# zcash/halo2

Measured on NVIDIA H100. Metric: msm_pairs_per_s, higher is better.
Workload: dtype u32x8 (255-bit modular integers)

## Files before the change

halo2_b200/csrc/capi_msm.cu:

```cuda
#define H2_MSM_QUAD_ACCUM_REFS (g_ctx.small_accum_refs)
#include "util_kernels.cuh"
#include "msm.cuh"
#include "ipa.cuh"
#include "ntt.cuh"
#include "ecfft.cuh"
#include "fixedbase.cuh"
static_assert(H2_FB_BITS == H2_FB_BITS_CTX, "ctx.cuh: fixed_table");


static int exclusive_scan_u32(uint32_t *d, uint64_t n, cudaStream_t s, const uint32_t *only_if = nullptr) {
    const uint64_t per_block = (uint64_t)H2_SCAN_BLOCK * H2_SCAN_ITEMS;
    uint32_t nb = (uint32_t)((n + per_block - 1) / per_block);
    if (g_ctx.scan_blocks.ensure((size_t)nb * 4 + 16)) return 1;
    uint32_t *bs = g_ctx.scan_blocks.as<uint32_t>();
    LAUNCH(scan_block_sums_kernel, nb, H2_SCAN_BLOCK, 0, s, d, n, bs, only_if);
    LAUNCH(scan_single_block_kernel, 1, H2_SCAN_BLOCK, 0, s, bs, nb, only_if);
    LAUNCH(scan_apply_kernel, nb, H2_SCAN_BLOCK, 0, s, d, n, bs, only_if);
    return 0;
}

uint32_t g_chunk_cut[H2_MAX_UPLOAD_CHUNKS + 1][H2_MAX_UPLOAD_CHUNKS + 1] = {
    {0, 16, 16, 16, 16}, {0, 16, 16, 16, 16}, {0, 4, 16, 16, 16}, {0, 2, 8, 16, 16}, {0, 1, 4, 10, 16}};
static inline size_t chunk_first(size_t n, uint32_t k, uint32_t j) {
    const auto &cut = g_chunk_cut;
// ... 28 lines not shown
        ge = &X.graphs.back();
    }
    ge->stamp = ++X.graph_stamp;
    if (ge->exec) {
        CU(cudaGraphLaunch(ge->exec, s));
        g_launches.fetch_add(ge->launches, std::memory_order_relaxed);
        return 0;
    }
    if (ge->seen++ == 0) return issue();
    const uint64_t l0 = g_launches.load();
    if (cudaStreamBeginCapture(s, cudaStreamCaptureModeThreadLocal) != cudaSuccess) { cudaGetLastError(); return issue(); }
    int rc = issue();
    cudaGraph_t graph = nullptr;
    cudaError_t ce = cudaStreamEndCapture(s, &graph);
    if (rc || ce != cudaSuccess || !graph) {
        if (graph) cudaGraphDestroy(graph);
        cudaGetLastError();
        ge->seen = 0;
        return rc ? rc : issue();
    }
    ge->launches = g_launches.load() - l0;
    ce = cudaGraphInstantiate(&ge->exec, graph, 0);
    cudaGraphDestroy(graph);
    if (ce != cudaSuccess) { ge->exec = nullptr; cudaGetLastError(); return issue(); }
    CU(cudaGraphLaunch(ge->exec, s));
    return 0;
}

template <class P, class PS>
static int msm_run(const fe *d_scalars, int scalars_mont, const affine *d_bases, size_t n, uint32_t c, uint32_t fixed, uint64_t stride,
                   jacobian *d_out, int out_canonical, cudaStream_t s, const BasesChunks *bc = nullptr, uint32_t sets = 1) {
    Context &X = g_ctx;
    if (n == 0) {
        jacobian id;
        id.x = fe_zero(); id.y = out_canonical ? fe_zero() : fe_one<P>(); id.z = fe_zero();
        if (out_canonical) id.y.v[0] = 1;
        std::vector<jacobian> ids(sets ? sets : 1u, id);
        CU(cudaMemcpyAsync(d_out, ids.data(), ids.size() * sizeof id, cudaMemcpyHostToDevice, s));
        CU(cudaStreamSynchronize(s));
        return 0;
    }
    std::function<int()> issue;
    auto record = [&X](uint32_t mode, uint32_t c_, uint32_t W, uint32_t sets_, uint32_t accum, uint32_t natural, uint32_t fast) {
        const uint32_t v[8] = {mode, c_, W, sets_, accum, natural, fast, X.fast_retry ? 1u : 0u};
        memcpy(X.last_plan, v, sizeof v);
        X.have_plan = true;
    };
    if (fixed == 2) {
        FbPlan fp;
        fp.total = n; fp.sets = sets ? sets : 1u; fp.split = fb_split(n, fp.sets); fp.scalars_mont = scalars_mont ? 1u : 0u;
        record(2, H2_FB_BITS, H2_FB_WINDOWS, fp.sets, 2, 0, 0);
        const uint64_t count0 = n * fp.split;
        if (X.fb_a.ensure(fp.sets * count0 * sizeof(xyzz)) || X.fb_b.ensure(fp.sets * fb_ctas(count0, fb_fan(count0)) * sizeof(xyzz))) return 1;
        issue = [&X, fp, count0, d_scalars, d_bases, d_out, out_canonical, s]() -> int {
            auto k_acc = fb_accum_kernel<P, PS>;
            auto k_red = fb_reduce_kernel<P, PS>;
            xyzz *a = X.fb_a.as<xyzz>(), *b = X.fb_b.as<xyzz>();
            prof_begin(PROF_MSM_ACCUM0, s);
            LAUNCH(k_acc, blocks_for(fp.sets * count0, 128), 128, 0, s, fp, d_scalars, d_bases, a);
            prof_end(s);
            uint64_t count = count0, in_stride = count0;
            for (;;) {
                const uint32_t f = fb_fan(count);
                const uint64_t ctas = fb_ctas(count, f);
                LAUNCH(k_red, dim3((unsigned)ctas, fp.sets), 4 * H2_FB_QUADS, 0, s, (const xyzz *)a, count, in_stride, f, b, ctas,
                       ctas == 1 ? d_out : (jacobian *)nullptr, (uint32_t)out_canonical);
                if (ctas == 1) break;
                xyzz *t = a; a = b; b = t;
                count = ctas; in_stride = ctas;
            }
            return 0;
        };
        return msm_issue_or_replay(issue, !bc, d_scalars, d_bases, d_out, n, stride, H2_FB_BITS, fp.sets, scalars_mont, out_canonical, s);
    }
    const uint32_t glv = (!fixed && X.glv_on && n < (1ull << 30)) ? 1u : 0u;
    if (c == 0) c = X.window_override ? X.window_override : msm_default_window(n, glv);
    if (c > 24) return fail("msm: window bits > 24");
    const uint32_t K = (bc && !fixed && bc->k > 1) ? bc->k : 1u;
    const uint32_t force_cap = X.sort_bins ? 0u : H2_MSM_NO_BINS;
    MsmPlan p;
    msm_make_plan(p, n, c, 0, 0, fixed, stride, glv, sets, force_cap);
    p.chunks = K;
    p.fast = (fixed == 1 && !bc && X.fast_now && p.cap != 0) ? 1u : 0u;
    X.last_fast = p.fast != 0;
    if (p.fast && p.T < p.cap) { p.T = p.cap; p.acc_chunk[0] = p.T; }
    p.natural = (p.fast && p.G <= X.natural_max_buckets && p.max_refs <= 2 * H2_MSM_QUAD_ACCUM_REFS && (X.accum_ways <= 1 || X.accum_ways >= 12)) ? 1u : 0u;
    MsmPlan pk[H2_MAX_UPLOAD_CHUNKS];
    size_t first[H2_MAX_UPLOAD_CHUNKS + 1];
    for (uint32_t j = 0; j <= K; j++) first[j] = chunk_first(n, K, j);
    uint64_t ref_space = 0, max_items = 0, part_total = 0;
    uint32_t t_max = 0;
    for (uint32_t j = 0; j < K; j++) {
        if (K == 1) pk[0] = p;
        else msm_make_plan(pk[j], first[j + 1] - first[j], c, 0, 0, fixed, stride, glv, sets, force_cap);
        if (pk[j].ref_space >= (1ull << 32)) return fail("msm: n * windows exceeds 2^32 references");
        ref_space = pk[j].ref_space > ref_space ? pk[j].ref_space : ref_space;
        max_items = pk[j].max_items > max_items ? pk[j].max_items : max_items;
        part_total = pk[j].part_total > part_total ? pk[j].part_total : part_total;
        t_max = pk[j].T > t_max ? pk[j].T : t_max;
    }
    bool thread_per_item = false;
    for (uint32_t j = 0; j < K; j++) thread_per_item |= pk[j].max_refs > (pk[j].fixed ? 2 : 1) * H2_MSM_QUAD_ACCUM_REFS;
    record(fixed, c, p.W, p.sets, thread_per_item ? 1u : 0u, p.natural, p.fast);
    uint64_t ba_space = 0;
    if (!fixed && X.ba_rounds) {
        size_t free_b = 0, total_b = 0;
        CU(cudaMemGetInfo(&free_b, &total_b));
        for (uint32_t j = 0; j < K; j++) {
            if (pk[j].max_refs > H2_MSM_QUAD_ACCUM_REFS && (uint64_t)K * pk[j].ref_space * 56 <= free_b / 2) msm_plan_ba(pk[j], X.ba_rounds, X.ba_target);
            if (pk[j].ba) ba_space = pk[j].ref_space > ba_space ? pk[j].ref_space : ba_space;
        }
    }
    if (K == 1) p.ba = pk[0].ba;
    if (ba_space)
        for (uint32_t r = 0; r < H2_BA_MAX_ROUNDS; r++)
            if (X.ba_lv[r].ensure(K * ((ba_space >> (r + 1)) + 1) * sizeof(affine))) return 1;
    if (glv && (X.bases_phi.ensure(n * sizeof(affine)) || X.glv_parts.ensure(n * 32))) return 1;
    if (fixed && (uint64_t)p.W * stride >= (1ull << 31)) return fail("msm: window table too large for 31-bit references");
    if (p.G >= (1ull << 32) || n >= (1ull << 31)) return fail("msm: n * windows exceeds 2^32 references");
    if (scalars_mont && X.scal_canon.ensure(n * p.sets * sizeof(fe))) return 1;
    const size_t small_words = 2 * (t_max + 2) + 8;
    part_total += 1;
    if (X.counts.ensure(K * (p.G + 1) * 4) || X.cursor.ensure(K * 2 * p.G * 4) || X.refs.ensure(K * ref_space * 4) ||
        X.size_hist.ensure(K * small_words * 4) || X.items.ensure(K * max_items * sizeof(uint2)) ||
        X.bucket_sum.ensure(K * p.G * sizeof(xyzz)) || X.pkey.ensure(K * part_total * 4) || X.pstart.ensure(K * part_total * 4) ||
        X.pend.ensure(K * part_total * 4) || X.ppt.ensure(K * part_total * sizeof(xyzz)) ||
        X.ra_t.ensure((size_t)p.Wb * p.m1 * sizeof(xyzz)) || X.ra_e.ensure((size_t)p.Wb * p.m1 * sizeof(xyzz)) ||
        X.r0.ensure((size_t)p.Wb * p.nb0 * H2_R0_ROWS * sizeof(xyzz)) || X.r1.ensure((size_t)p.Wb * p.r1_rows * sizeof(xyzz)) ||
        X.wsum.ensure((size_t)p.Wb * sizeof(xyzz)))
        return 1;
    MsmBuffers Mk[H2_MAX_UPLOAD_CHUNKS];
    for (uint32_t j = 0; j < K; j++) {
        MsmBuffers &M = Mk[j];
        const size_t o = first[j];
        M.scalars = d_scalars + o; M.bases = d_bases + o; M.bases_phi = X.bases_phi.as<affine>() + o;
        M.glv_parts = X.glv_parts.as<uint32_t>() + 8 * o; M.scalars_mont = scalars_mont ? 1u : 0u;
        M.scal_canon = X.scal_canon.as<fe>() + o;
        M.counts = X.counts.as<uint32_t>() + j * (p.G + 1); M.cursor = X.cursor.as<uint32_t>() + j * 2 * p.G; M.cursor2 = M.cursor + p.G;
        M.refs = X.refs.as<uint32_t>() + j * ref_space;
        M.size_hist = X.size_hist.as<uint32_t>() + j * small_words; M.size_cursor = M.size_hist + (pk[j].T + 2); M.flags = M.size_cursor + (pk[j].T + 2);
        M.items = X.items.as<uint2>() + j * max_items;
        M.bucket_sum = X.bucket_sum.as<xyzz>() + j * p.G;
        for (uint32_t r = 0; r < H2_BA_MAX_ROUNDS; r++) M.ba[r] = ba_space ? X.ba_lv[r].as<affine>() + j * ((ba_space >> (r + 1)) + 1) : nullptr;
        M.pkey = X.pkey.as<uint32_t>() + j * part_total; M.pstart = X.pstart.as<uint32_t>() + j * part_total;
        M.pend = X.pend.as<uint32_t>() + j * part_total; M.ppt = X.ppt.as<xyzz>() + j * part_total;
        M.ra_t = X.ra_t.as<xyzz>(); M.ra_e = X.ra_e.as<xyzz>(); M.r0 = X.r0.as<xyzz>(); M.r1 = X.r1.as<xyzz>();
        M.wsum = X.wsum.as<xyzz>(); M.result = d_out;
    }
    X.last_flags = Mk[0].flags;

    {
        const uint64_t per_block = (uint64_t)H2_SCAN_BLOCK * H2_SCAN_ITEMS;
        if (X.scan_blocks.ensure((size_t)((p.G + 1 + per_block - 1) / per_block) * 4 + 16)) return 1;
    }
    issue = [&]() -> int {
        if (!p.fast) CU(cudaMemsetAsync(X.counts.p, 0, K * (p.G + 1) * 4, s));
        CU(cudaMemsetAsync(X.cursor.p, 0, K * 2 * p.G * 4, s));
        CU(cudaMemsetAsync(X.size_hist.p, 0, K * small_words * 4, s));
        CU(cudaMemsetAsync(X.bucket_sum.p, 0, K * p.G * sizeof(xyzz), s));
        if (!p.fast) CU(cudaMemsetAsync(X.pkey.p, 0xff, K * part_total * 4, s));

        auto k_bin = msm_bin_kernel<P, PS>;
        auto k_hist = msm_hist_kernel<P, PS>;
        auto k_scatter = msm_scatter_kernel<P, PS>;
        auto k_ihist = msm_item_hist_kernel<P, PS>;
        auto k_ibases = msm_item_bases_kernel<P, PS>;
        auto k_iplace = msm_item_place_kernel<P, PS>;
        auto k_accum0 = msm_accum0_kernel<P, PS>;
        auto k_accum0q = msm_accum0_quad_kernel<P, PS>;
        auto k_accum0p2 = msm_accum0_pair_kernel<P, PS>;
        auto k_accum0s2 = msm_accum0_split_kernel<P, PS, 2>;
        auto k_accum0s4 = msm_accum0_split_kernel<P, PS, 4>;
        auto k_accum0m2 = msm_accum0_multi_kernel<P, PS, 2>;
        auto k_accum0m4 = msm_accum0_multi_kernel<P, PS, 4>;
        auto k_ba = X.ba_variant == 1 ? msm_ba_round_kernel<P, PS, 4, 5> : X.ba_variant == 2 ? msm_ba_round_kernel<P, PS, 2, 4>
                  : X.ba_variant == 3 ? msm_ba_round_kernel<P, PS, 2, 5> : msm_ba_round_kernel<P, PS, 4, 4>;
        auto k_accum0p = msm_accum0_pts_kernel<P, PS>;
        auto k_accumN = msm_accumN_kernel<P, PS>;
        auto k_rest = msm_accum_rest_kernel<P, PS>;
        auto k_reduceA = msm_reduceA_kernel<P, PS>;
        auto k_r0 = msm_r0_kernel<P, PS>;
        auto k_r1 = msm_r1_kernel<P, PS>;
        auto k_wsum = msm_wsum_kernel<P, PS>;
        auto k_final = msm_final_kernel<P, PS>;
        for (uint32_t j = 0; j < K; j++) {
            const MsmPlan &q = pk[j];
            const MsmBuffers &M = Mk[j];
            if (bc && bc->k) {
                for (uint32_t e = (K > 1 ? j : 0); e < (K > 1 ? j + 1 : bc->k); e++) {
                    if (bc->wait_recorded(2 * e + 1)) return fail("msm: the upload of the inputs failed");
                    CU(cudaStreamWaitEvent(s, bc->ev_scal[e], 0));
                }
            }
            if (q.cap == 0) CU(cudaMemsetAsync(M.flags + 1, 0x01, 4, s));
            else LAUNCH(k_bin, blocks_for(q.n * q.sets, 256), 256, 0, s, q, M);
            if (!q.fast) {
                LAUNCH(k_hist, blocks_for(q.n * q.sets, 256), 256, 0, s, q, M);
                if (exclusive_scan_u32(M.counts, q.G + 1, s, M.flags + 1)) return 1;
                LAUNCH(k_scatter, blocks_for(q.n * q.sets, 256), 256, 0, s, q, M);
            }
            if (!q.natural) {
                LAUNCH(k_ihist, blocks_for(q.G, 256), 256, 0, s, q, M);
                LAUNCH(k_ibases, 1, 32, 0, s, q, M);
                LAUNCH(k_iplace, blocks_for(q.G, 256), 256, 0, s, q, M);
            }
            if (bc && bc->k) {
                for (uint32_t e = (K > 1 ? j : 0); e < (K > 1 ? j + 1 : bc->k); e++) {
                    if (bc->wait_recorded(2 * e + 2)) return fail("msm: the upload of the inputs failed");
                    CU(cudaStreamWaitEvent(s, bc->ev[e], 0));
                }
            }
            if (q.glv) {
                auto k_phi = msm_phi_kernel<P, PS>;
                LAUNCH(k_phi, blocks_for(q.n, 256), 256, 0, s, M.bases, M.bases_phi, (uint64_t)q.n);
            }
            prof_begin(PROF_MSM_ACCUM0, s);
            if (q.max_refs <= (q.fixed ? 2 : 1) * H2_MSM_QUAD_ACCUM_REFS) {
                if (X.accum_ways == 4) LAUNCH(k_accum0m4, blocks_for(q.max_items * 16, 128), 128, 0, s, q, M);
                else if (X.accum_ways == 2) LAUNCH(k_accum0m2, blocks_for(q.max_items * 8, 128), 128, 0, s, q, M);
                else if (X.accum_ways == 0) LAUNCH(k_accum0p2, blocks_for(q.max_items * 2, 128), 128, 0, s, q, M);
                else if (X.accum_ways == 12) LAUNCH(k_accum0s2, blocks_for(q.max_items * 2, 128), 128, 0, s, q, M);
                else if (X.accum_ways == 14) LAUNCH(k_accum0s4, blocks_for(q.max_items * 4, 128), 128, 0, s, q, M);
                else LAUNCH(k_accum0q, blocks_for(q.max_items * 4, 128), 128, 0, s, q, M);
            }
            else {
                for (uint32_t r = 1; r <= q.ba; r++)
                    LAUNCH(k_ba, blocks_for((q.max_items + q.ba_m[r - 1] - 1) / q.ba_m[r - 1], 128), 128, 0, s, q, M, r);
                if (q.ba) LAUNCH(k_accum0p, blocks_for(q.max_items, 128), 128, 0, s, q, M);
                LAUNCH(k_accum0, blocks_for(q.max_items, 128), 128, 0, s, q, M);
            }
            prof_end(s);
            if (!q.fast) {
                if (q.acc_levels > 1) LAUNCH(k_accumN, blocks_for(q.acc_threads[1], 128), 128, 0, s, q, M, 1u);
                if (q.acc_levels > 2) LAUNCH(k_accumN, blocks_for(q.acc_threads[2], 128), 128, 0, s, q, M, 2u);
                if (q.acc_levels > 3) LAUNCH(k_rest, 1, 256, 0, s, q, M);
            }
        }
        const MsmBuffers &M = Mk[0];
        LAUNCH(k_reduceA, blocks_for((uint64_t)p.Wb * p.m1 * 4, 128), 128, 0, s, p, M);
        LAUNCH(k_r0, blocks_for((uint64_t)p.Wb * p.nb0 * (2 + p.bits0) * 4, 128), 128, 0, s, p, M);
        LAUNCH(k_r1, p.Wb * p.r1_rows, 4 * H2_R1_QUADS, 0, s, p, M);
        LAUNCH(k_wsum, p.Wb, 128, 0, s, p, M);
        LAUNCH(k_final, 1, 64, 0, s, p, M, (uint32_t)out_canonical);
        return 0;
    };
    return msm_issue_or_replay(issue, fixed && !bc, d_scalars, d_bases, d_out, n, stride, c, sets, scalars_mont, out_canonical, s);
}

int msm_dispatch(int curve, const fe *d_scalars, int scalars_mont, const affine *d_bases, size_t n, uint32_t c,
                 jacobian *d_out, int out_canonical, cudaStream_t s, uint32_t fixed, uint64_t stride,
                 const BasesChunks *bc, uint32_t sets) {
    if (curve == H2_CURVE_PALLAS) return msm_run<FpParams, FqParams>(d_scalars, scalars_mont, d_bases, n, c, fixed, stride, d_out, out_canonical, s, bc, sets);
    if (curve == H2_CURVE_VESTA) return msm_run<FqParams, FpParams>(d_scalars, scalars_mont, d_bases, n, c, fixed, stride, d_out, out_canonical, s, bc, sets);
    return fail("unknown curve id");
}
int fixed_pass_flags(cudaStream_t s) {
    Context &X = g_ctx;
    if (!X.last_fast) return 0;
    if (!X.h_flags) CU(cudaHostAlloc((void **)&X.h_flags, 2 * sizeof(uint32_t), cudaHostAllocDefault));
    CU(cudaMemcpyAsync(X.h_flags, X.last_flags, 2 * sizeof(uint32_t), cudaMemcpyDeviceToHost, s));
    return 0;
}
bool fixed_pass_ok() {
    Context &X = g_ctx;
    return !X.last_fast || (X.h_flags[0] == 0 && X.h_flags[1] == 0);
}
static uint32_t table_window(size_t n) {
    uint32_t lg = 0;
    while ((1ull << (lg + 1)) <= n) lg++;
    uint32_t want = lg + 2;
    if (want <= 9) return 8;
    if (want <= 15) return 15;
    if (want == 16) return 15;
    if (want <= 18) return 16;
    if (want <= 20) return 17;
    return 20;
}
static int build_table(BaseSet *b, uint32_t c, cudaStream_t s) {
    if (c == 0) c = table_window(b->n);
    if (c < 4 || c > 24) return fail("window table: window bits must be in [4, 24]");
    uint32_t W = (256 + c - 1) / c;
    if ((uint64_t)W * b->n >= (1ull << 31)) return fail("window table: too many points");
    if (b->table.ensure((size_t)W * b->n * sizeof(affine))) return 1;
    if (b->curve == H2_CURVE_PALLAS) {
        auto k = msm_table_kernel<FpParams, FqParams>;
        LAUNCH(k, blocks_for(b->n, 128), 128, 0, s, b->buf.as<affine>(), b->table.as<affine>(), (uint64_t)b->n, (uint64_t)b->n, c, W);
    } else {
// ... 653 lines not shown
```

halo2_b200/csrc/msm.cuh:

```cuda
#pragma once
#include "curve.cuh"
#include "glv.cuh"

namespace h2 {

H2_HD affine ld_affine(const affine *p) { affine r; r.x = fe_load(&p->x); r.y = fe_load(&p->y); return r; }
H2_HD void st_affine(affine *p, const affine &a) { fe_store(&p->x, a.x); fe_store(&p->y, a.y); }
H2_HD xyzz ld_xyzz(const xyzz *p) { xyzz r; r.x = fe_load(&p->x); r.y = fe_load(&p->y); r.zz = fe_load(&p->zz); r.zzz = fe_load(&p->zzz); return r; }
H2_HD void st_xyzz(xyzz *p, const xyzz &a) { fe_store(&p->x, a.x); fe_store(&p->y, a.y); fe_store(&p->zz, a.zz); fe_store(&p->zzz, a.zzz); }
H2_HD void st_jacobian(jacobian *p, const jacobian &a) { fe_store(&p->x, a.x); fe_store(&p->y, a.y); fe_store(&p->z, a.z); }

#define H2_MSM_INVALID_KEY 0xffffffffu
#define H2_MSM_MAX_LEVELS 12
#define H2_R0_LOG 3
#define H2_R0_ROWS 5

struct MsmPlan {
    uint64_t n;
    uint32_t c;
    uint32_t glv;
    uint32_t chunks;
    uint32_t cap;
    uint32_t cap_top;
    uint64_t g_top;
// ... 184 lines not shown
    static H2_HD void load_scalar(const MsmBuffers &M, uint64_t i, uint32_t (&s)[8], bool first_pass) {
        fe x;
        if (M.scalars_mont) {
            if (first_pass) { x = fe_from_mont<PS>(fe_load(M.scalars + i)); fe_store(M.scal_canon + i, x); }
            else x = fe_load(M.scal_canon + i);
        } else x = fe_load(M.scalars + i);
        for (int k = 0; k < 8; k++) s[k] = x.v[k];
    }

    static H2_HD void load_parts(const MsmPlan &p, const MsmBuffers &M, uint64_t i, bool first_pass, uint32_t (&part)[2][8], uint32_t (&neg)[2]) {
        neg[0] = neg[1] = 0;
        if (!p.glv) { uint32_t s[8]; load_scalar(M, i, s, first_pass); for (int k = 0; k < 8; k++) part[0][k] = s[k]; return; }
        uint4 *q = reinterpret_cast<uint4 *>(M.glv_parts) + i * 2;
        if (first_pass) {
            uint32_t s[8];
            load_scalar(M, i, s, true);
            glv_decompose<P>(s, part[0], neg[0], part[1], neg[1]);
            for (int e = 0; e < 2; e++)
                q[e] = make_uint4(part[e][0], part[e][1], part[e][2], part[e][3] | (neg[e] << 31));
        } else {
            for (int e = 0; e < 2; e++) {
                uint4 v = q[e];
                part[e][0] = v.x; part[e][1] = v.y; part[e][2] = v.z; part[e][3] = v.w & 0x7fffffffu; neg[e] = v.w >> 31;
                part[e][4] = part[e][5] = part[e][6] = part[e][7] = 0;
            }
        }
    }

    template <class F> static H2_HD bool for_each_digit(const MsmPlan &p, const MsmBuffers &M, uint64_t i, bool first_pass, F &&f) {
        uint32_t part[2][8], neg[2];
        const uint32_t halves = p.glv ? 2u : 1u;
        load_parts(p, M, i, first_pass, part, neg);
        bool ok = true;
        for (uint32_t e = 0; e < halves; e++) {
            uint32_t carry = 0;
            for (uint32_t w = 0; w < p.W; w++) {
                int32_t d = next_digit(part[e], w, p.c, carry);
                if (d == 0) continue;
                uint32_t mag = d < 0 ? (uint32_t)(-d) : (uint32_t)d;
                uint32_t g = (uint32_t)((uint64_t)(p.fixed ? i / p.n : w) * p.B + (mag - 1));
                uint32_t ref = (uint32_t)(p.fixed ? i % p.n + (uint64_t)w * p.stride : i);
                ref |= (e << 30) | ((((uint32_t)(d < 0)) ^ neg[e]) << 31);
                f(g, ref);
            }
            ok = ok && carry == 0;
        }
        return ok;
    }

    static H2_HD uint64_t item_slot(const MsmPlan &p, uint32_t start, bool first_piece) {
        return 2ull * (start / p.T) + (first_piece ? 1 : 0);
    }
    static H2_HD bool bin_of(const MsmPlan &p, uint64_t g, uint32_t &lo, uint32_t &cap) {
        if (g < p.g_top) { lo = (uint32_t)(g * p.cap); cap = p.cap; return true; }
        const uint64_t b = g - p.g_top;
        lo = (uint32_t)(p.g_top * p.cap + b * p.cap_top); cap = p.cap_top;
        return b < p.top_bins;
    }
    static H2_HD uint32_t bucket_lo(const MsmPlan &p, const MsmBuffers &M, uint64_t g) {
        if (M.flags[1]) return M.counts[g];
        uint32_t lo, cap;
        return bin_of(p, g, lo, cap) ? lo : 0u;
    }
    static H2_HD uint32_t bucket_hi(const MsmPlan &p, const MsmBuffers &M, uint64_t g) {
        if (M.flags[1]) return M.counts[g + 1];
        uint32_t lo, cap;
        return bin_of(p, g, lo, cap) ? lo + M.cursor[g] : 0u;
    }
    static H2_HD void count_items(const MsmPlan &p, const MsmBuffers &M, uint64_t g, uint32_t &nfull, uint32_t &rem) {
        uint32_t cnt = bucket_hi(p, M, g) - bucket_lo(p, M, g);
        nfull = cnt / p.T; rem = cnt % p.T;
        if (cnt > p.T) M.flags[0] = 1;
    }
    static H2_HD void size_bases_body(const MsmPlan &p, const MsmBuffers &M) {
        uint32_t run = 0;
        for (uint32_t sz = p.T; sz >= 1; sz--) {
            uint32_t c = M.size_hist[sz];
            M.size_cursor[sz] = run;
            run += c;
        }
        M.size_cursor[0] = run;
        M.size_hist[p.T + 1] = run;
    }

    struct Flusher {
        const MsmBuffers *M;
        const MsmPlan *p;
        H2_HD void flush(uint32_t g, uint32_t a, uint32_t b, const xyzz &acc, uint64_t slot) {
            uint32_t lo = bucket_lo(*p, *M, g), hi = bucket_hi(*p, *M, g);
            if (a == lo && b == hi) {
                st_xyzz(M->bucket_sum + g, acc);
            } else {
                M->pkey[slot] = g; M->pstart[slot] = a; M->pend[slot] = b;
                st_xyzz(M->ppt + slot, acc);
            }
        }
    };

    struct BaItem { uint32_t in_base, out_base, len, np; };
    static H2_HD BaItem ba_item(const MsmPlan &p, const MsmBuffers &M, uint32_t r, uint64_t t) {
        const uint2 it = M.items[t];
        const uint32_t hi = bucket_hi(p, M, it.x), end = it.y + p.T < hi ? it.y + p.T : hi;
        BaItem b;
        b.len = (end - it.y + (1u << (r - 1)) - 1u) >> (r - 1);
        b.np = b.len >> 1; b.in_base = it.y >> (r - 1); b.out_base = it.y >> r;
        return b;
    }
    static H2_HD const affine *ba_addr(const MsmPlan &p, const MsmBuffers &M, uint32_t r, uint32_t key) {
        if (r > 1) return M.ba[r - 2] + key;
        if (p.glv) return ((key >> 30) & 1u ? M.bases_phi : M.bases) + (key & 0x3fffffffu);
        return M.bases + (key & 0x7fffffffu);
    }
    static H2_HD affine ba_load(const MsmPlan &p, const MsmBuffers &M, uint32_t r, uint32_t key) {
        affine b = ld_affine(ba_addr(p, M, r, key));
        if (r == 1 && (key >> 31)) b.y = fe_neg<P>(b.y);
        return b;
    }
    static H2_HD uint32_t ba_key(const MsmBuffers &M, uint32_t r, uint32_t idx) { return r == 1 ? M.refs[idx] : idx; }
    static H2_HD void ba_prefetch(const void *q) {
#ifdef __CUDA_ARCH__
        asm volatile("prefetch.global.L1 [%0];" ::"l"(q));
#else
        (void)q;
#endif
    }
    static H2_HD uint32_t ba_kind(const affine &A, const affine &B, fe &d) {
        d = fe_sub<P>(B.x, A.x);
        if (!fe_is_zero(d) && !fe_is_zero(A.x) && !fe_is_zero(B.x)) return 0;
        if (affine_is_identity(A) || affine_is_identity(B)) { d = fe_one<P>(); return 1; }
        if (!fe_is_zero(d)) return 0;
        if (fe_eq(A.y, B.y)) { d = fe_dbl<P>(A.y); return 2; }
        d = fe_one<P>();
        return 3;
    }
    template <int U> static H2_HD void ba_batch(const MsmPlan &p, const MsmBuffers &M, uint32_t r, uint64_t ta, uint64_t tb, bool single,
                                                 uint32_t k_lo, uint32_t k_hi, fe *pre) {
        affine *out = M.ba[r - 1];
        fe acc = fe_one<P>();
        uint32_t c = 0;
        for (uint64_t tt = ta; tt < tb; tt++) {
            const BaItem it = ba_item(p, M, r, tt);
            const uint32_t ka = single ? k_lo : 0u, kb = single ? k_hi : it.np;
            for (uint32_t k = ka; k < kb; k += U) {
                uint32_t key[2 * U];
#pragma unroll
                for (int u = 0; u < 2 * U; u++) key[u] = 2 * k + u < 2 * kb ? ba_key(M, r, it.in_base + 2 * k + u) : 0u;
#pragma unroll
                for (int u = 0; u < 2 * U; u++) if (2 * k + u < 2 * kb) ba_prefetch(ba_addr(p, M, r, key[u]));
#pragma unroll
                for (int u = 0; u < U; u++) {
                    if (k + u >= kb) break;
                    const fe x1 = fe_load(&ba_addr(p, M, r, key[2 * u])->x), x2 = fe_load(&ba_addr(p, M, r, key[2 * u + 1])->x);
                    fe d = fe_sub<P>(x2, x1);
                    if (fe_is_zero(d) || fe_is_zero(x1) || fe_is_zero(x2)) { affine A = ba_load(p, M, r, key[2 * u]), B = ba_load(p, M, r, key[2 * u + 1]); ba_kind(A, B, d); }
                    pre[c++] = acc;
                    acc = fe_mul_call<P>(acc, d);
                }
            }
        }
        if (c == 0) return;
        fe inv = fe_inv_gcd<P>(acc);
        for (uint64_t tt = tb; tt-- > ta;) {
            const BaItem it = ba_item(p, M, r, tt);
            const uint32_t ka = single ? k_lo : 0u, kb = single ? k_hi : it.np;
            if (kb <= ka) continue;
            for (uint32_t k = ka + ((kb - ka - 1) / U) * U;; k -= U) {
// ... 265 lines not shown
    for (uint32_t e = 0; e < halves; e++) {
        uint32_t carry = 0;
        for (uint32_t w0 = 0; w0 < p.W; w0 += 4) {
            uint32_t slot[4], gid[4], ref[4];
            bool act[4];
#pragma unroll
            for (int k = 0; k < 4; k++) {
                uint32_t w = w0 + k;
                int32_t d = w < p.W ? Msm<P, PS>::next_digit(part[e], w, p.c, carry) : 0;
                act[k] = in && d != 0;
                uint32_t mag = d < 0 ? (uint32_t)(-d) : (uint32_t)d;
                gid[k] = (uint32_t)((uint64_t)(p.fixed ? set : (w < p.W ? w : 0)) * p.B + (act[k] ? mag - 1 : 0));
                ref[k] = ((uint32_t)idx + (uint32_t)(p.fixed && w < p.W ? (uint64_t)w * p.stride : 0)) | (e << 30) |
                         ((((uint32_t)(d < 0)) ^ sneg[e]) << 31);
                slot[k] = warp_inc<true>(M.cursor + gid[k], act[k]);
            }
#pragma unroll
            for (int k = 0; k < 4; k++)
                if (act[k]) {
                    uint32_t lo, cap;
                    if (Msm<P, PS>::bin_of(p, gid[k], lo, cap) && slot[k] < cap) M.refs[lo + slot[k]] = ref[k];
                    else full = true;
                }
        }
    }
    if (full) M.flags[1] = 1;
}
template <class P, class PS> __global__ void __launch_bounds__(256) msm_hist_kernel(const MsmPlan p, const MsmBuffers M) {
    if (!M.flags[1]) return;
    uint64_t i = (uint64_t)blockIdx.x * blockDim.x + threadIdx.x;
    bool in = i < p.n * p.sets;
    const uint64_t set = p.fixed && in ? i / p.n : 0;
    uint32_t part[2][8] = {{0, 0, 0, 0, 0, 0, 0, 0}, {0, 0, 0, 0, 0, 0, 0, 0}}, sneg[2] = {0, 0};
    const uint32_t halves = p.glv ? 2u : 1u;
    if (in) Msm<P, PS>::load_parts(p, M, i, true, part, sneg);
    for (uint32_t e = 0; e < halves; e++) {
        uint32_t carry = 0;
        for (uint32_t w = 0; w < p.W; w++) {
            int32_t d = Msm<P, PS>::next_digit(part[e], w, p.c, carry);
            bool act = in && d != 0;
            uint32_t mag = d < 0 ? (uint32_t)(-d) : (uint32_t)d;
            uint64_t g = (uint64_t)(p.fixed ? set : w) * p.B + (act ? mag - 1 : 0);
            warp_inc<false>(M.counts + g, act);
        }
    }
}
template <class P, class PS> __global__ void __launch_bounds__(256) msm_scatter_kernel(const MsmPlan p, const MsmBuffers M) {
    if (!M.flags[1]) return;
    uint64_t i = (uint64_t)blockIdx.x * blockDim.x + threadIdx.x;
    bool in = i < p.n * p.sets;
    const uint64_t set = p.fixed && in ? i / p.n : 0, idx = p.fixed && in ? i % p.n : i;
    uint32_t part[2][8] = {{0, 0, 0, 0, 0, 0, 0, 0}, {0, 0, 0, 0, 0, 0, 0, 0}}, sneg[2] = {0, 0};
    const uint32_t halves = p.glv ? 2u : 1u;
    if (in) Msm<P, PS>::load_parts(p, M, i, false, part, sneg);
    for (uint32_t e = 0; e < halves; e++) {
        uint32_t carry = 0;
        for (uint32_t w0 = 0; w0 < p.W; w0 += 4) {
            uint32_t slot[4], gid[4], ref[4];
            bool act[4];
#pragma unroll
            for (int k = 0; k < 4; k++) {
                uint32_t w = w0 + k;
                int32_t d = w < p.W ? Msm<P, PS>::next_digit(part[e], w, p.c, carry) : 0;
                act[k] = in && d != 0;
                uint32_t mag = d < 0 ? (uint32_t)(-d) : (uint32_t)d;
                gid[k] = (uint32_t)((uint64_t)(p.fixed ? set : (w < p.W ? w : 0)) * p.B + (act[k] ? mag - 1 : 0));
                ref[k] = ((uint32_t)idx + (uint32_t)(p.fixed && w < p.W ? (uint64_t)w * p.stride : 0)) | (e << 30) |
                         ((((uint32_t)(d < 0)) ^ sneg[e]) << 31);
                slot[k] = warp_inc<true>(M.cursor2 + gid[k], act[k]);
            }
#pragma unroll
            for (int k = 0; k < 4; k++)
                if (act[k]) M.refs[M.counts[gid[k]] + slot[k]] = ref[k];
        }
    }
}
template <class P, class PS> __global__ void __launch_bounds__(256) msm_phi_kernel(const affine *bases, affine *out, uint64_t n) {
    uint64_t i = (uint64_t)blockIdx.x * blockDim.x + threadIdx.x;
    if (i >= n) return;
    affine b = ld_affine(bases + i);
    b.x = fe_mul<P>(b.x, glv_zeta<P>());
    st_affine(out + i, b);
}
template <class P, class PS> __global__ void __launch_bounds__(256) msm_item_hist_kernel(const MsmPlan p, const MsmBuffers M) {
    if (p.fast && M.flags[1]) return;
    uint64_t g = (uint64_t)blockIdx.x * blockDim.x + threadIdx.x;
    uint32_t nfull = 0, rem = 0;
    if (g < p.G) Msm<P, PS>::count_items(p, M, g, nfull, rem);
    if (nfull) atomicAdd(M.size_hist + p.T, nfull);
    warp_inc<false>(M.size_hist + rem, rem != 0);
}
template <class P, class PS> __global__ void msm_item_bases_kernel(const MsmPlan p, const MsmBuffers M) {
    if (threadIdx.x == 0 && blockIdx.x == 0) Msm<P, PS>::size_bases_body(p, M);
}
template <class P, class PS> __global__ void __launch_bounds__(256) msm_item_place_kernel(const MsmPlan p, const MsmBuffers M) {
    if (p.fast && M.flags[1]) return;
    uint64_t g = (uint64_t)blockIdx.x * blockDim.x + threadIdx.x;
    uint32_t nfull = 0, rem = 0, lo = 0;
    if (g < p.G) { Msm<P, PS>::count_items(p, M, g, nfull, rem); lo = Msm<P, PS>::bucket_lo(p, M, g); }
    if (nfull) {
        uint32_t at = atomicAdd(M.size_cursor + p.T, nfull);
        for (uint32_t k = 0; k < nfull; k++) M.items[at + k] = make_uint2((uint32_t)g, lo + k * p.T);
    }
    uint32_t at = warp_inc<true>(M.size_cursor + rem, rem != 0);
    if (rem) M.items[at] = make_uint2((uint32_t)g, lo + nfull * p.T);
}
template <class P, class PS> __global__ void __launch_bounds__(128) msm_table_kernel(const affine *bases, affine *table, uint64_t count, uint64_t stride,
                                                                                    uint32_t c, uint32_t W) {
    Msm<P, PS>::table_body(bases, table, count, stride, c, W, (uint64_t)blockIdx.x * blockDim.x + threadIdx.x);
}
template <class P, class PS> __global__ void __launch_bounds__(128, 5) msm_accum0_kernel(const MsmPlan p, const MsmBuffers M) {
    uint64_t t = (uint64_t)blockIdx.x * blockDim.x + threadIdx.x;
    Msm<P, PS>::accum0_body(p, M, t);
}
template <class P, class PS, int U, int MINB> __global__ void __launch_bounds__(128, MINB) msm_ba_round_kernel(const MsmPlan p, const MsmBuffers M, uint32_t r) {
    Msm<P, PS>::template ba_round_body<128, U>(p, M, r, (uint64_t)blockIdx.x * blockDim.x + threadIdx.x);
}
template <class P, class PS> __global__ void __launch_bounds__(128, 5) msm_accum0_pts_kernel(const MsmPlan p, const MsmBuffers M) {
    Msm<P, PS>::accum0_pts_body(p, M, (uint64_t)blockIdx.x * blockDim.x + threadIdx.x);
}
template <class P, class PS> __global__ void __launch_bounds__(128) msm_accum0_quad_kernel(const MsmPlan p, const MsmBuffers M) {
    uint64_t t = ((uint64_t)blockIdx.x * blockDim.x + threadIdx.x) >> 2;
    Msm<P, PS>::template accum0_body<QuadAdd, true>(p, M, t);
}
template <class P, class PS> __global__ void __launch_bounds__(128) msm_accum0_pair_kernel(const MsmPlan p, const MsmBuffers M) {
    uint64_t t = ((uint64_t)blockIdx.x * blockDim.x + threadIdx.x) >> 1;
    Msm<P, PS>::template accum0_body<PairAdd, true>(p, M, t);
}
template <class P, class PS, int WAYS> __global__ void __launch_bounds__(128) msm_accum0_multi_kernel(const MsmPlan p, const MsmBuffers M) {
    const uint64_t t = ((uint64_t)blockIdx.x * blockDim.x + threadIdx.x) / (4 * WAYS);
    if (p.fast && M.flags[1]) return;
    if (t >= M.size_hist[p.T + 1]) return;
    const uint32_t lane = threadIdx.x & 31u, h = (lane >> 2) & (WAYS - 1);
    const uint32_t gmask = (WAYS == 8 ? 0xffffffffu : ((1u << (4 * WAYS)) - 1u) << (lane & ~(4u * WAYS - 1u)));
    const uint2 it = M.items[t];
    const uint32_t g = it.x, start = it.y, lo = Msm<P, PS>::bucket_lo(p, M, g), hi = Msm<P, PS>::bucket_hi(p, M, g);
    const uint32_t end = start + p.T < hi ? start + p.T : hi;
    xyzz acc = xyzz_identity();
    for (uint32_t pos = start + h; pos < end; pos += WAYS) {
        const uint32_t ref = M.refs[pos];
        affine b;
        if (p.glv) b = ld_affine(((ref >> 30) & 1u ? M.bases_phi : M.bases) + (ref & 0x3fffffffu));
        else b = ld_affine(M.bases + (ref & 0x7fffffffu));
        if (ref >> 31) b.y = fe_neg<P>(b.y);
        xyzz_add_mixed_quad<P>(acc, b);
    }
#pragma unroll
    for (int step = WAYS / 2; step >= 1; step >>= 1) {
        xyzz other;
#pragma unroll
        for (int i = 0; i < 8; i++) {
            other.x.v[i] = __shfl_down_sync(gmask, acc.x.v[i], 4 * step, 4 * WAYS);
            other.y.v[i] = __shfl_down_sync(gmask, acc.y.v[i], 4 * step, 4 * WAYS);
            other.zz.v[i] = __shfl_down_sync(gmask, acc.zz.v[i], 4 * step, 4 * WAYS);
            other.zzz.v[i] = __shfl_down_sync(gmask, acc.zzz.v[i], 4 * step, 4 * WAYS);
        }
        if ((int)h < step) xyzz_add_quad<P>(acc, other);
    }
    if (h == 0) {
        typename Msm<P, PS>::Flusher F; F.M = &M; F.p = &p;
        F.flush(g, start, end, acc, p.part_offset[1] + Msm<P, PS>::item_slot(p, start, start == lo));
    }
}
template <class P, class PS, int WAYS> __global__ void __launch_bounds__(128) msm_accum0_split_kernel(const MsmPlan p, const MsmBuffers M) {
    const uint64_t t = ((uint64_t)blockIdx.x * blockDim.x + threadIdx.x) / WAYS;
    if (p.fast && M.flags[1]) return;
    const uint32_t lane = threadIdx.x & 31u, h = lane & (WAYS - 1);
    uint2 it;
    bool live = true;
    if (p.natural) {
        live = t < p.G;
        it = make_uint2((uint32_t)(live ? t : 0), live ? Msm<P, PS>::bucket_lo(p, M, live ? t : 0) : 0u);
    } else {
        live = t < M.size_hist[p.T + 1];
        it = live ? M.items[t] : make_uint2(0u, 0u);
    }
    const uint32_t g = it.x, start = it.y, lo = Msm<P, PS>::bucket_lo(p, M, g), hi = live ? Msm<P, PS>::bucket_hi(p, M, g) : start;
    const uint32_t end = start + p.T < hi ? start + p.T : hi;
    xyzz acc = xyzz_identity();
    if (start + h < end) {
        uint32_t ref = M.refs[start + h];
        affine nxt = Msm<P, PS>::ref_point(p, M, ref);
        for (uint32_t pos = start + h; pos < end; pos += WAYS) {
            affine b = nxt;
            const uint32_t neg = ref >> 31;
            if (pos + WAYS < end) { ref = M.refs[pos + WAYS]; nxt = Msm<P, PS>::ref_point(p, M, ref); }
            if (neg) b.y = fe_neg<P>(b.y);
            xyzz_add_mixed<P>(acc, b);
// ... 187 lines not shown
```

Measured before the change: 242.3 million.

## Aggregate MSM item-size histogram in shared memory and fuse size-base scan into placement

Item histogram and placement kernels now process several buckets per thread and accumulate per-size counts in shared memory, issuing one global atomic per size per block instead of per-thread atomics. The single-thread size-bases kernel is removed; each placement block recomputes the size offsets with a block-wide scan over the histogram. Bucket-sum zeroing for non-natural plans moves from a full memset into the placement kernel, which clears only empty buckets. The fast path is disabled when cap exceeds a new size limit, and plans with more sizes than that limit now fail.

```diff
diff --git a/halo2_b200/csrc/capi_msm.cu b/halo2_b200/csrc/capi_msm.cu
--- a/halo2_b200/csrc/capi_msm.cu
+++ b/halo2_b200/csrc/capi_msm.cu
@@ -134,9 +134,10 @@
     msm_make_plan(p, n, c, 0, 0, fixed, stride, glv, sets, force_cap);
     p.chunks = K;
     p.fast = (fixed == 1 && !bc && X.fast_now && p.cap != 0) ? 1u : 0u;
+    p.natural = (p.fast && p.G <= X.natural_max_buckets && p.max_refs <= 2 * H2_MSM_QUAD_ACCUM_REFS && (X.accum_ways <= 1 || X.accum_ways >= 12)) ? 1u : 0u;
+    if (p.fast && !p.natural && p.cap > H2_MSM_ITEM_SIZES) p.fast = 0;
+    if (p.fast && p.T < p.cap) { p.T = p.cap; p.acc_chunk[0] = p.T; }
     X.last_fast = p.fast != 0;
-    if (p.fast && p.T < p.cap) { p.T = p.cap; p.acc_chunk[0] = p.T; }
-    p.natural = (p.fast && p.G <= X.natural_max_buckets && p.max_refs <= 2 * H2_MSM_QUAD_ACCUM_REFS && (X.accum_ways <= 1 || X.accum_ways >= 12)) ? 1u : 0u;
     MsmPlan pk[H2_MAX_UPLOAD_CHUNKS];
     size_t first[H2_MAX_UPLOAD_CHUNKS + 1];
     for (uint32_t j = 0; j <= K; j++) first[j] = chunk_first(n, K, j);
@@ -171,6 +172,7 @@
     if (fixed && (uint64_t)p.W * stride >= (1ull << 31)) return fail("msm: window table too large for 31-bit references");
     if (p.G >= (1ull << 32) || n >= (1ull << 31)) return fail("msm: n * windows exceeds 2^32 references");
     if (scalars_mont && X.scal_canon.ensure(n * p.sets * sizeof(fe))) return 1;
+    if (!p.natural && t_max > H2_MSM_ITEM_SIZES) return fail("msm: work items of more than H2_MSM_ITEM_SIZES references");
     const size_t small_words = 2 * (t_max + 2) + 8;
     part_total += 1;
     if (X.counts.ensure(K * (p.G + 1) * 4) || X.cursor.ensure(K * 2 * p.G * 4) || X.refs.ensure(K * ref_space * 4) ||
@@ -209,14 +211,13 @@
         if (!p.fast) CU(cudaMemsetAsync(X.counts.p, 0, K * (p.G + 1) * 4, s));
         CU(cudaMemsetAsync(X.cursor.p, 0, K * 2 * p.G * 4, s));
         CU(cudaMemsetAsync(X.size_hist.p, 0, K * small_words * 4, s));
-        CU(cudaMemsetAsync(X.bucket_sum.p, 0, K * p.G * sizeof(xyzz), s));
+        if (p.natural) CU(cudaMemsetAsync(X.bucket_sum.p, 0, K * p.G * sizeof(xyzz), s));
         if (!p.fast) CU(cudaMemsetAsync(X.pkey.p, 0xff, K * part_total * 4, s));
 
         auto k_bin = msm_bin_kernel<P, PS>;
         auto k_hist = msm_hist_kernel<P, PS>;
         auto k_scatter = msm_scatter_kernel<P, PS>;
         auto k_ihist = msm_item_hist_kernel<P, PS>;
-        auto k_ibases = msm_item_bases_kernel<P, PS>;
         auto k_iplace = msm_item_place_kernel<P, PS>;
         auto k_accum0 = msm_accum0_kernel<P, PS>;
         auto k_accum0q = msm_accum0_quad_kernel<P, PS>;
@@ -252,9 +253,9 @@
                 LAUNCH(k_scatter, blocks_for(q.n * q.sets, 256), 256, 0, s, q, M);
             }
             if (!q.natural) {
-                LAUNCH(k_ihist, blocks_for(q.G, 256), 256, 0, s, q, M);
-                LAUNCH(k_ibases, 1, 32, 0, s, q, M);
-                LAUNCH(k_iplace, blocks_for(q.G, 256), 256, 0, s, q, M);
+                const uint32_t item_blocks = blocks_for(q.G, H2_ITEM_THREADS * H2_ITEM_BUCKETS);
+                LAUNCH(k_ihist, item_blocks, H2_ITEM_THREADS, (q.T + 1) * 4, s, q, M);
+                LAUNCH(k_iplace, item_blocks, H2_ITEM_THREADS, 2 * (q.T + 1) * 4, s, q, M);
             }
             if (bc && bc->k) {
                 for (uint32_t e = (K > 1 ? j : 0); e < (K > 1 ? j + 1 : bc->k); e++) {
diff --git a/halo2_b200/csrc/msm.cuh b/halo2_b200/csrc/msm.cuh
--- a/halo2_b200/csrc/msm.cuh
+++ b/halo2_b200/csrc/msm.cuh
@@ -290,6 +290,14 @@
         M.size_cursor[0] = run;
         M.size_hist[p.T + 1] = run;
     }
+    static H2_HD void place_items(const MsmPlan &p, const MsmBuffers &M, uint64_t g, uint32_t nfull, uint32_t rem, uint32_t at_full, uint32_t at_rem) {
+        const uint32_t lo = bucket_lo(p, M, g);
+        for (uint32_t k = 0; k < nfull; k++) M.items[at_full + k] = make_uint2((uint32_t)g, lo + k * p.T);
+        if (rem) M.items[at_rem] = make_uint2((uint32_t)g, lo + nfull * p.T);
+    }
+    static H2_HD void clear_sum_word(const MsmBuffers &M, uint64_t g, uint32_t w) {
+        reinterpret_cast<uint4 *>(M.bucket_sum + g)[w] = make_uint4(0u, 0u, 0u, 0u);
+    }
 
     struct Flusher {
         const MsmBuffers *M;
@@ -721,28 +729,88 @@
     b.x = fe_mul<P>(b.x, glv_zeta<P>());
     st_affine(out + i, b);
 }
-template <class P, class PS> __global__ void __launch_bounds__(256) msm_item_hist_kernel(const MsmPlan p, const MsmBuffers M) {
+#define H2_ITEM_THREADS 256
+#define H2_ITEM_BUCKETS 4
+#define H2_MSM_ITEM_SIZES 4096u
+template <class P, class PS> __global__ void __launch_bounds__(H2_ITEM_THREADS) msm_item_hist_kernel(const MsmPlan p, const MsmBuffers M) {
     if (p.fast && M.flags[1]) return;
-    uint64_t g = (uint64_t)blockIdx.x * blockDim.x + threadIdx.x;
-    uint32_t nfull = 0, rem = 0;
-    if (g < p.G) Msm<P, PS>::count_items(p, M, g, nfull, rem);
-    if (nfull) atomicAdd(M.size_hist + p.T, nfull);
-    warp_inc<false>(M.size_hist + rem, rem != 0);
-}
-template <class P, class PS> __global__ void msm_item_bases_kernel(const MsmPlan p, const MsmBuffers M) {
-    if (threadIdx.x == 0 && blockIdx.x == 0) Msm<P, PS>::size_bases_body(p, M);
-}
-template <class P, class PS> __global__ void __launch_bounds__(256) msm_item_place_kernel(const MsmPlan p, const MsmBuffers M) {
+    extern __shared__ uint32_t cnt[];
+    for (uint32_t s = threadIdx.x; s <= p.T; s += blockDim.x) cnt[s] = 0;
+    __syncthreads();
+    const uint64_t g0 = (uint64_t)blockIdx.x * (H2_ITEM_THREADS * H2_ITEM_BUCKETS) + threadIdx.x;
+    for (uint32_t k = 0; k < H2_ITEM_BUCKETS; k++) {
+        const uint64_t g = g0 + (uint64_t)k * H2_ITEM_THREADS;
+        if (g >= p.G) break;
+        uint32_t nfull, rem;
+        Msm<P, PS>::count_items(p, M, g, nfull, rem);
+        if (nfull) atomicAdd(cnt + p.T, nfull);
+        if (rem) atomicAdd(cnt + rem, 1u);
+    }
+    __syncthreads();
+    for (uint32_t s = threadIdx.x + 1; s <= p.T; s += blockDim.x)
+        if (cnt[s]) atomicAdd(M.size_hist + s, cnt[s]);
+}
+__device__ __forceinline__ uint32_t msm_item_size_offsets(const uint32_t *hist, uint32_t T, uint32_t *base, uint32_t *warp_tot) {
+    const uint32_t per = (T + blockDim.x - 1) / blockDim.x, q0 = threadIdx.x * per, q1 = q0 + per < T ? q0 + per : T;
+    uint32_t sum = 0;
+    for (uint32_t q = q0; q < q1; q++) sum += hist[T - q];
+    const uint32_t lane = threadIdx.x & 31u, wid = threadIdx.x >> 5;
+    uint32_t inc = sum;
+#pragma unroll
+    for (uint32_t o = 1; o < 32; o <<= 1) {
+        const uint32_t v = __shfl_up_sync(0xffffffffu, inc, o);
+        if (lane >= o) inc += v;
+    }
+    if (lane == 31) warp_tot[wid] = inc;
+    __syncthreads();
+    uint32_t run = inc - sum, total = 0;
+    for (uint32_t w = 0; w < (blockDim.x >> 5); w++) {
+        const uint32_t t = warp_tot[w];
+        if (w < wid) run += t;
+        total += t;
+    }
+    for (uint32_t q = q0; q < q1; q++) {
+        const uint32_t s = T - q;
+        base[s] = run;
+        run += hist[s];
+    }
+    __syncthreads();
+    return total;
+}
+template <class P, class PS> __global__ void __launch_bounds__(H2_ITEM_THREADS) msm_item_place_kernel(const MsmPlan p, const MsmBuffers M) {
     if (p.fast && M.flags[1]) return;
-    uint64_t g = (uint64_t)blockIdx.x * blockDim.x + threadIdx.x;
-    uint32_t nfull = 0, rem = 0, lo = 0;
-    if (g < p.G) { Msm<P, PS>::count_items(p, M, g, nfull, rem); lo = Msm<P, PS>::bucket_lo(p, M, g); }
-    if (nfull) {
-        uint32_t at = atomicAdd(M.size_cursor + p.T, nfull);
-        for (uint32_t k = 0; k < nfull; k++) M.items[at + k] = make_uint2((uint32_t)g, lo + k * p.T);
-    }
-    uint32_t at = warp_inc<true>(M.size_cursor + rem, rem != 0);
-    if (rem) M.items[at] = make_uint2((uint32_t)g, lo + nfull * p.T);
+    extern __shared__ uint32_t sh[];
+    uint32_t *base = sh, *cnt = sh + (p.T + 1);
+    __shared__ uint32_t warp_tot[H2_ITEM_THREADS / 32];
+    __shared__ uint8_t empty[H2_ITEM_THREADS * H2_ITEM_BUCKETS];
+    for (uint32_t s = threadIdx.x; s <= p.T; s += blockDim.x) cnt[s] = 0;
+    const uint32_t total = msm_item_size_offsets(M.size_hist, p.T, base, warp_tot);
+    if (blockIdx.x == 0 && threadIdx.x == 0) M.size_hist[p.T + 1] = total;
+    const uint64_t g0 = (uint64_t)blockIdx.x * (H2_ITEM_THREADS * H2_ITEM_BUCKETS) + threadIdx.x;
+    uint32_t nfull[H2_ITEM_BUCKETS], rem[H2_ITEM_BUCKETS], rfull[H2_ITEM_BUCKETS], rrem[H2_ITEM_BUCKETS];
+#pragma unroll
+    for (uint32_t k = 0; k < H2_ITEM_BUCKETS; k++) {
+        const uint64_t g = g0 + (uint64_t)k * H2_ITEM_THREADS;
+        nfull[k] = rem[k] = rfull[k] = rrem[k] = 0;
+        if (g < p.G) {
+            Msm<P, PS>::count_items(p, M, g, nfull[k], rem[k]);
+            if (nfull[k]) rfull[k] = atomicAdd(cnt + p.T, nfull[k]);
+            if (rem[k]) rrem[k] = atomicAdd(cnt + rem[k], 1u);
+        }
+        empty[k * H2_ITEM_THREADS + threadIdx.x] = g < p.G && !nfull[k] && !rem[k];
+    }
+    __syncthreads();
+    for (uint32_t s = threadIdx.x + 1; s <= p.T; s += blockDim.x)
+        if (cnt[s]) base[s] += atomicAdd(M.size_cursor + s, cnt[s]);
+    const uint64_t tile = (uint64_t)blockIdx.x * (H2_ITEM_THREADS * H2_ITEM_BUCKETS);
+    for (uint32_t j = threadIdx.x; j < H2_ITEM_THREADS * H2_ITEM_BUCKETS * 8; j += H2_ITEM_THREADS)
+        if (empty[j >> 3]) Msm<P, PS>::clear_sum_word(M, tile + (j >> 3), j & 7u);
+    __syncthreads();
+#pragma unroll
+    for (uint32_t k = 0; k < H2_ITEM_BUCKETS; k++) {
+        const uint64_t g = g0 + (uint64_t)k * H2_ITEM_THREADS;
+        if (g < p.G) Msm<P, PS>::place_items(p, M, g, nfull[k], rem[k], base[p.T] + rfull[k], rem[k] ? base[rem[k]] + rrem[k] : 0u);
+    }
 }
 template <class P, class PS> __global__ void __launch_bounds__(128) msm_table_kernel(const affine *bases, affine *table, uint64_t count, uint64_t stride,
                                                                                     uint32_t c, uint32_t W) {
```

After: 246.3 million, median of 6. 1.6% higher.
